# codebydant/sfM_danPipeline

Measured on AMD Instinct MI355X. Metric: image-pairs matched/sec + BA iterations/sec (200 cams, 100k pts, 1M obs), higher is better.
Workload: dtype i8

## Files before the change

### sfm_danpipeline_amd/csrc/match.hip

```cpp
#include "common.h"
#include <type_traits>
#include <vector>
#include <algorithm>
#include <string.h>
#include <stdlib.h>

namespace {

typedef int v4i __attribute__((ext_vector_type(4)));
typedef int v16i __attribute__((ext_vector_type(16)));

enum { KIND_F32_L2 = 0, KIND_U8_L2 = 1, KIND_U8_HAMMING = 2 };

constexpr int TILE_ROWS = 32;
constexpr int HPAD = -(1 << 23);
constexpr int TAG_BITS = 8;
constexpr int EPOCH_TILES = 1 << TAG_BITS;
constexpr int TAG_MASK = EPOCH_TILES - 1;
constexpr int FIX_FLAG = 1 << 30;
constexpr int FIX_GRID = 1024;
constexpr int FIX_CAP = 1 << 20;
constexpr int DIST_EMPTY = 0x7FFFFFFF;
constexpr int KNN_WAVES = 4;
constexpr int HCHUNK = 1024;
// ... 192 lines not shown
      }
    }
#pragma unroll
    for (int e = 0; e < 16; ++e) {
      const int k = c * 16 + e;
      int x = 128;
      if (valid && k < dim) {
        if (KIND == KIND_F32_L2) {
          const float f = fv[e];
          ok = ok && (f == rintf(f)) && (f >= 0.f) && (f <= 255.f);
          x = (int)f;
          x = x < 0 ? 0 : (x > 255 ? 255 : x);
        } else {
          x = bv[e];
        }
      }
      const int cv = x - 128;
      v[e] = (signed char)cv;
      n2 += cv * cv;
    }
  }
#pragma unroll
  for (int o = 1; o < NC; o <<= 1) n2 += __shfl_xor(n2, o);
  int4 out;
  memcpy(&out, v, 16);
  int4* dst = (int4*)(I.tiles + (size_t)tile * (TILE_ROWS * RB)) + chunk_pos<NC>(r, c);
  *dst = out;
  if (c == 0) {
    int ci;
    if (KIND == KIND_U8_HAMMING)
      ci = ((valid ? dim * 8 * (HCHUNK / 2) : (dim * 8 + 1) * HCHUNK)) | (pos & (HCHUNK - 1));
    else ci = valid ? -((n2 + 1) >> 1) : HPAD;
    I.cin[pos] = ci;
    I.nq[pos] = valid ? n2 : 0;
  }
  if (KIND == KIND_F32_L2 && !ok) nonintegral[img] = gen;
}

template <int NC>
__device__ __forceinline__ int group_sum(int x) {
  if (NC >= 2) x += __builtin_amdgcn_update_dpp(0, x, 0xB1, 0xF, 0xF, true);
  if (NC >= 4) x += __builtin_amdgcn_update_dpp(0, x, 0x4E, 0xF, 0xF, true);
  if (NC >= 8) x += __builtin_amdgcn_update_dpp(0, x, 0x141, 0xF, 0xF, true);
  if (NC >= 16) x += __builtin_amdgcn_update_dpp(0, x, 0x140, 0xF, 0xF, true);
  return x;
}

struct Best2 {
  int d0, i0, x0, d1, i1, x1;
};
__device__ __forceinline__ bool lex_less(int da, int ia, int db, int ib) { return da < db || (da == db && ia < ib); }
__device__ __forceinline__ void best2_insert(Best2& b, int d, int i, int x) {
  if (lex_less(d, i, b.d0, b.i0)) {
    b.d1 = b.d0;
    b.i1 = b.i0;
    b.x1 = b.x0;
    b.d0 = d;
    b.i0 = i;
    b.x0 = x;
  } else if (lex_less(d, i, b.d1, b.i1)) {
    b.d1 = d;
    b.i1 = i;
    b.x1 = x;
  }
}

template <int I>
__device__ __forceinline__ void epi_op(const v16i& D0, const v16i& D1, int (&sl)[16], int& k0, int& k1, int (&T)[16],
                                       int tag0, int tag1) {
  if constexpr (I < 16) {
    sl[I] = imax3(sl[I], D0[I], D1[I]);
  } else {
    constexpr int J = (I - 16) % 11;
    constexpr int B = (I - 16) < 11 ? 0 : 8;
    const v16i& D = (I - 16) < 11 ? D0 : D1;
    const int tag = (I - 16) < 11 ? tag0 : tag1;
    if constexpr (J == 0) T[B + 0] = imax3(D[0], D[1], D[2]);
    if constexpr (J == 1) T[B + 1] = imax3(D[3], D[4], D[5]);
    if constexpr (J == 2) T[B + 2] = imax3(D[6], D[7], D[8]);
    if constexpr (J == 3) T[B + 3] = imax3(D[9], D[10], D[11]);
    if constexpr (J == 4) T[B + 4] = imax3(D[12], D[13], D[14]);
    if constexpr (J == 5) T[B + 5] = imax3(T[B + 0], T[B + 1], T[B + 2]);
    if constexpr (J == 6) T[B + 6] = imax3(T[B + 3], T[B + 4], D[15]);
    if constexpr (J == 7) T[B + 7] = max(T[B + 5], T[B + 6]);
    if constexpr (J == 8) T[B + 7] = (T[B + 7] << TAG_BITS) | tag;
    if constexpr (J == 9) k1 = imed3(k0, k1, T[B + 7]);
    if constexpr (J == 10) k0 = max(k0, T[B + 7]);
  }
}
constexpr int EPI_ORDER[38] = {16, 17, 18, 19, 20, 21, 22, 23, 24, 25, 26, 27, 28, 29, 30, 31, 0, 1,  2,
                                          32, 33, 3,  4,  5,  34, 6,  7,  8,  9,  35, 10, 11, 12, 13, 36, 37, 14, 15};
template <int LO, int HI>
__device__ __forceinline__ void epi_range(const v16i& D0, const v16i& D1, int (&sl)[16], int& k0, int& k1, int (&T)[16],
                                          int tag0, int tag1) {
  if constexpr (LO < HI && LO < 38) {
    epi_op<EPI_ORDER[LO]>(D0, D1, sl, k0, k1, T, tag0, tag1);
    epi_range<LO + 1, HI>(D0, D1, sl, k0, k1, T, tag0, tag1);
  }
}

template <int KS, int MODE, int NU, int SR>
__global__ __launch_bounds__(KNN_WAVES * 64, 2) void knn_kernel(const ImgDev* __restrict__ imgs,
                                                         const WorkItem* __restrict__ items,
                                                         const int* __restrict__ nonintegral, int gen, int dim,
                                                         int4* __restrict__ knn, int maxq,
                                                         int* __restrict__ fix_count, int2* __restrict__ fix_items) {
  constexpr int NC = 2 * KS;
  constexpr int RB = 32 * KS;
  constexpr int TILE_BYTES = TILE_ROWS * RB;
  constexpr int STAGE_ROW_BYTES = SR * RB;
  constexpr int NW = KNN_WAVES;
  constexpr int NT = NW * 64;
  constexpr int CIN_COPIES = (SR + NT - 1) / NT;
  constexpr int STAGE_BYTES = STAGE_ROW_BYTES + CIN_COPIES * NT * 4;
  constexpr int TILES = SR / TILE_ROWS;
  constexpr int TP = TILES / 2;
  constexpr int PIECES = STAGE_ROW_BYTES / (NT * 16);
  constexpr int BATCH = KS <= 4 ? 4 : 2;
  constexpr int NG = 2 * KS;
  constexpr int STAGES_PER_EPOCH = EPOCH_TILES / TILES;
  static_assert(PIECES >= 1 && TP >= 2 && TP % 2 == 0 && STAGES_PER_EPOCH % 2 == 0, "stage shape");
  constexpr int SCRATCH_W = 2048 + (TILE_ROWS * RB > 4096 ? TILE_ROWS * RB : 4096);
  constexpr int BUFA_BYTES = STAGE_BYTES > NW * SCRATCH_W ? STAGE_BYTES : NW * SCRATCH_W;
  constexpr int BUFB_BYTES = (NU < 2 || STAGE_BYTES > NW * SCRATCH_W) ? STAGE_BYTES : NW * SCRATCH_W;
  __shared__ __attribute__((aligned(16))) unsigned char ldsA[BUFA_BYTES];
  __shared__ __attribute__((aligned(16))) unsigned char ldsB[BUFB_BYTES];

  const WorkItem it = items[blockIdx.x];
  if ((nonintegral[it.qimg] == gen) | (nonintegral[it.timg] == gen)) return;
  const ImgDev Q = imgs[it.qimg];
  const ImgDev T = imgs[it.timg];
  const int lane = threadIdx.x & 63;
  const int wave = __builtin_amdgcn_readfirstlane(threadIdx.x >> 6);
  const int r = lane & 31, h = lane >> 5;
  const int nqt = Q.n_pad / TILE_ROWS;
  int qt[NU], qtc[NU];
#pragma unroll
  for (int u = 0; u < NU; ++u) {
    qt[u] = it.qtile0 + NU * wave + u;
    qtc[u] = qt[u] < Q.n_pad / TILE_ROWS ? qt[u] : (Q.n_pad >= TILE_ROWS ? Q.n_pad / TILE_ROWS - 1 : 0);
  }
  SFM_STAMP(0);
  int dbg_trips = 0;

  v4i bq[NU][KS];
#pragma unroll
  for (int u = 0; u < NU; ++u) {
    g_v4i_p src = (g_v4i_p)(Q.tiles + (size_t)qtc[u] * TILE_BYTES);
#pragma unroll
    for (int ks = 0; ks < KS; ++ks) bq[u][ks] = src[chunk_pos<NC>(r, 2 * ks + h)];
  }

  int aoff[KS];
#pragma unroll
  for (int ks = 0; ks < KS; ++ks) aoff[ks] = chunk_pos<NC>(r, 2 * ks + h) * 16;
  const int coff = STAGE_ROW_BYTES + h * 16;

  const int nstages = T.n_pad / SR;
  const int tid = threadIdx.x;

  const __amdgpu_buffer_rsrc_t rs_tiles = __builtin_amdgcn_make_buffer_rsrc((void*)T.tiles, 0, 0x7FFFFFFF, 0x00020000);
  const __amdgpu_buffer_rsrc_t rs_cin = __builtin_amdgcn_make_buffer_rsrc((void*)T.cin, 0, 0x7FFFFFFF, 0x00020000);
  auto stage_copy = [&](int stage, unsigned char* dstb) {
    const int off = stage * STAGE_ROW_BYTES;
#if SFM_DBG == 6
    const unsigned char* src = (const unsigned char*)T.tiles + (size_t)stage * STAGE_ROW_BYTES;
#pragma unroll
    for (int i = 0; i < PIECES; ++i)
      __builtin_amdgcn_global_load_lds((const SFM_GLOBAL void*)(src + (size_t)(i * NT + tid) * 16),
                                       (__attribute__((address_space(3))) void*)(dstb + i * (NT * 16) + wave * 1024), 16, 0, 0);
#pragma unroll
    for (int i = 0; i < CIN_COPIES; ++i)
      __builtin_amdgcn_global_load_lds((const SFM_GLOBAL void*)(T.cin + (size_t)stage * SR + i * NT + tid),
                                       (__attribute__((address_space(3))) void*)(dstb + STAGE_ROW_BYTES + i * (NT * 4) + wave * 256), 4, 0, 0);
    (void)off;
#else
#pragma unroll
    for (int i = 0; i < PIECES; ++i)
      __builtin_amdgcn_raw_ptr_buffer_load_lds(rs_tiles, (__attribute__((address_space(3))) void*)(dstb + i * (NT * 16) + wave * 1024),
                                               16, (i * NT + tid) * 16, off, 0, 0);
#pragma unroll
    for (int i = 0; i < CIN_COPIES; ++i)
      __builtin_amdgcn_raw_ptr_buffer_load_lds(rs_cin, (__attribute__((address_space(3))) void*)(dstb + STAGE_ROW_BYTES + i * (NT * 4) + wave * 256),
                                               4, (i * NT + tid) * 4, stage * SR * 4, 0, 0);
#endif
  };
  auto ld_afrag = [&](const unsigned char* tb, int ks) -> v4i {
    const int4 x = *(const int4*)(tb + aoff[ks]);
    return v4i{x.x, x.y, x.z, x.w};
  };
  auto ld_cin = [&](const unsigned char* sb, int tl, v16i& C) {
#pragma unroll
    for (int g = 0; g < 4; ++g) {
      const int4 x = *(const int4*)(sb + coff + (tl * TILE_ROWS + 8 * g) * 4);
      C[4 * g] = x.x;
      C[4 * g + 1] = x.y;
      C[4 * g + 2] = x.z;
      C[4 * g + 3] = x.w;
    }
  };

  const int nodd_t = MODE == 0 ? *(g_i32_p)T.nodd : 0;
  const int nbits = dim * 8;

  for (int ep0 = 0; ep0 < nstages; ep0 += STAGES_PER_EPOCH) {
    const int ep1 = (ep0 + STAGES_PER_EPOCH < nstages) ? ep0 + STAGES_PER_EPOCH : nstages;
    const int ep_tile0 = ep0 * TILES;
    int sl[NU][16], k0[NU], k1[NU];
#pragma unroll
    for (int u = 0; u < NU; ++u) {
      k0[u] = k1[u] = (int)0x80000000;
#pragma unroll
      for (int e = 0; e < 16; ++e) sl[u][e] = HPAD;
    }
    if (ep0 > 0) __syncthreads();
    stage_copy(ep0, ldsA);
    asm volatile("s_waitcnt vmcnt(0)" ::: "memory");
    __syncthreads();

    v4i F0[KS], F1[KS];
    v16i C0, C1, X0, X1, Y0, Y1;
    int TT[16];
    {
      const unsigned char* sb = ldsA;
#pragma unroll
      for (int ks = 0; ks < KS; ++ks) F0[ks] = ld_afrag(sb, ks);
      ld_cin(sb, 0, C0);
#pragma unroll
      for (int e = 0; e < 16; ++e) X0[e] = X1[e] = Y0[e] = Y1[e] = HPAD;
    }
    int tag = EPOCH_TILES - 1 + 2;
    SFM_STAMP(1);

#define SFM_CHAIN(FA, FB, UF, DA, DB, UD, LD1, SB1, T1, LD0, SB0, T0)                                       \
  do {                                                                                                      \
    _Pragma("unroll") for (int g_ = 0; g_ < NG; ++g_) {                                                     \
      const int ks_ = g_ % KS;                                                                              \
      if (SFM_DBG == 3) {                                                                                   \
        if (g_ < KS) FA[ks_] += F0[ks_][0] + C0[ks_];                                                       \
        else FB[ks_] += F1[ks_][0] + C1[ks_];                                                               \
      } else if (g_ < KS) FA = __builtin_amdgcn_mfma_i32_32x32x32_i8(F0[ks_], bq[UF][ks_], ks_ == 0 ? C0 : FA, 0, 0, 0); \
      else FB = __builtin_amdgcn_mfma_i32_32x32x32_i8(F1[ks_], bq[UF][ks_], ks_ == 0 ? C1 : FB, 0, 0, 0);  \
      if ((LD1) && g_ == 0) {                                                                               \
        _Pragma("unroll") for (int k2_ = 0; k2_ < KS; ++k2_) F1[k2_] = ld_afrag((SB1) + (T1) * TILE_BYTES, k2_); \
        ld_cin(SB1, T1, C1);                                                                                \
      }                                                                                                     \
      if ((LD0) && g_ < KS) {                                                                               \
        F0[ks_] = ld_afrag((SB0) + (T0) * TILE_BYTES, ks_);                                                 \
        if (g_ == 0) ld_cin(SB0, T0, C0);                                                                   \
      }                                                                                                     \
      if (SFM_DBG != 2) switch (g_) {                                                                       \
        SFM_EPI_CASES(DA, DB, UD)                                                                           \
      }                                                                                                     \
      __builtin_amdgcn_sched_barrier(0);                                                                    \
    }                                                                                                       \
  } while (0)
#define SFM_EPI_CASE(G, DA, DB, UD) \
  case G: epi_range<(G) * 38 / NG, ((G) + 1) * 38 / NG>(DA, DB, sl[UD], k0[UD], k1[UD], TT, tag & TAG_MASK, (tag - 1) & TAG_MASK); break;
#define SFM_EPI_CASES(DA, DB, UD)                                                                          \
  SFM_EPI_CASE(0, DA, DB, UD) SFM_EPI_CASE(1, DA, DB, UD) SFM_EPI_CASE(2, DA, DB, UD) SFM_EPI_CASE(3, DA, DB, UD)     \
  SFM_EPI_CASE(4, DA, DB, UD) SFM_EPI_CASE(5, DA, DB, UD) SFM_EPI_CASE(6, DA, DB, UD) SFM_EPI_CASE(7, DA, DB, UD)     \
  SFM_EPI_CASE(8, DA, DB, UD) SFM_EPI_CASE(9, DA, DB, UD) SFM_EPI_CASE(10, DA, DB, UD) SFM_EPI_CASE(11, DA, DB, UD)   \
  SFM_EPI_CASE(12, DA, DB, UD) SFM_EPI_CASE(13, DA, DB, UD) SFM_EPI_CASE(14, DA, DB, UD) SFM_EPI_CASE(15, DA, DB, UD)

    auto stage = [&](int s, const unsigned char* sb, unsigned char* nb) __attribute__((always_inline)) {
      const bool more = s + 1 < ep1;
      if (more) stage_copy(s + 1, nb);
#pragma unroll
      for (int tp = 0; tp < TP; ++tp) {
        const bool last = tp == TP - 1;
        if (NU == 2) {
          SFM_CHAIN(X0, X1, 0, Y0, Y1, 1, true, sb, 2 * tp + 1, false, sb, 0);
          tag -= 2;
          if (last) {
            asm volatile("s_waitcnt vmcnt(0)" ::: "memory");
            __syncthreads();
          }
          SFM_CHAIN(Y0, Y1, NU - 1, X0, X1, 0, false, sb, 0, true, last ? nb : sb, last ? 0 : 2 * tp + 2);
        } else {
          if (last) {
#pragma unroll
            for (int k2 = 0; k2 < KS; ++k2) F1[k2] = ld_afrag(sb + (2 * tp + 1) * TILE_BYTES, k2);
            ld_cin(sb, 2 * tp + 1, C1);
            asm volatile("s_waitcnt vmcnt(0)" ::: "memory");
            __syncthreads();
          }
          if ((tp & 1) == 0) SFM_CHAIN(X0, X1, 0, Y0, Y1, 0, !last, sb, 2 * tp + 1, true, last ? nb : sb, last ? 0 : 2 * tp + 2);
          else SFM_CHAIN(Y0, Y1, 0, X0, X1, 0, !last, sb, 2 * tp + 1, true, last ? nb : sb, last ? 0 : 2 * tp + 2);
          tag -= 2;
        }
      }
    
    };
    for (int s = ep0; s < ep1; s += 2) {
      stage(s, ldsA, ldsB);
      if (s + 1 < ep1) stage(s + 1, ldsB, ldsA);
    }
    SFM_STAMP(2);
    epi_range<0, 38>(Y0, Y1, sl[NU - 1], k0[NU - 1], k1[NU - 1], TT, tag & TAG_MASK, (tag - 1) & TAG_MASK);
#undef SFM_CHAIN
#undef SFM_EPI_CASES
#undef SFM_EPI_CASE

    int lane_p = lane;
    asm volatile("" : "+v"(lane_p));
    const int r_p = lane_p & 31, h_p = lane_p >> 5;
    typedef __attribute__((address_space(3))) int* lds_vi_p;
#define SFM_WAVE_LDS_FENCE() do { __builtin_amdgcn_fence(__ATOMIC_RELEASE, "wavefront"); __builtin_amdgcn_wave_barrier(); __builtin_amdgcn_fence(__ATOMIC_ACQUIRE, "wavefront"); } while (0)
    __attribute__((address_space(3))) unsigned char* wq[NU];
#pragma unroll
    for (int u = 0; u < NU; ++u)
      wq[u] = (__attribute__((address_space(3))) unsigned char*)(u == 0 ? ldsA : ldsB) + wave * SCRATCH_W + 2048;
    const lds_vi_p wl = (lds_vi_p)(wq[0] - 2048);
    const lds_vi_p wr = NU == 1 ? wl + 256 : (lds_vi_p)(wq[NU - 1] - 2048);
#pragma unroll
    for (int u = 0; u < NU; ++u)
#pragma unroll
      for (int ks = 0; ks < KS; ++ks)
        *(__attribute__((address_space(3))) v4i*)(wq[u] + chunk_pos<NC>(r_p, 2 * ks + h_p) * 16) = bq[u][ks];
    constexpr int SH = (NC == 16) ? 0 : (NC == 8) ? 1 : (NC == 4) ? 2 : 3;
    int cpos[NU][4], chv[NU][4], slot_[NU][4], count[NU];
    bool cval[NU][4], cload[NU][4];
    int qrow[NU], nqq[NU];
    int ovf[NU];
#pragma unroll
    for (int u = 0; u < NU; ++u) {
      const int q = qtc[u] * TILE_ROWS + r_p;
      qrow[u] = ((g_i32_p)Q.perm)[q];
      nqq[u] = ((g_i32_p)Q.nq)[q];
      if (qt[u] >= nqt) qrow[u] = -1;
    }
#pragma unroll
    for (int u = 0; u < NU; ++u) {
      const int bv0 = k0[u] >> TAG_BITS, bv1 = k1[u] >> TAG_BITS;
      const int tl0 = ep_tile0 + (EPOCH_TILES - 1) - (k0[u] & TAG_MASK);
      const int tl1 = ep_tile0 + (EPOCH_TILES - 1) - (k1[u] & TAG_MASK);
      const int pb0 = __shfl_xor(bv0, 32), pb1 = __shfl_xor(bv1, 32);
      int a0 = (HPAD - 1) * 16, a1 = a0, a2 = a0;
#pragma unroll
      for (int e = 0; e < 16; ++e) {
        const int key = (int)((unsigned)sl[u][e] << 4) | e;
        a2 = imed3(a1, a2, key);
        a1 = imed3(a0, a1, key);
        a0 = max(a0, key);
      }
      const int S0 = a0 >> 4, S1 = a1 >> 4, S2 = a2 >> 4;
      const int e0 = a0 & 15, e1 = a1 & 15;
      const int thr = max(max(min(bv0, pb0), max(bv1, pb1)), S1);
      const int ns = (S0 >= thr ? 1 : 0) + (S1 >= thr ? 1 : 0) + (S2 >= thr ? 1 : 0);
      const bool t0in = bv0 >= thr && bv0 > HPAD, t1in = bv1 >= thr && bv1 > HPAD;
      const int rho0 = 8 * (e0 >> 2) + 4 * h_p + (e0 & 3), rho1 = ns >= 2 ? 8 * (e1 >> 2) + 4 * h_p + (e1 & 3) : rho0;
      int over = (ns > 2 && (t0in || t1in)) ? 1 : 0;
      over |= __shfl_xor(over, 32);
      ovf[u] = over;
      const bool known = ns == 1;
      cpos[u][0] = tl0 * TILE_ROWS + rho0;
      cpos[u][1] = tl0 * TILE_ROWS + rho1;
      cpos[u][2] = tl1 * TILE_ROWS + rho0;
      cpos[u][3] = tl1 * TILE_ROWS + rho1;
      cval[u][0] = t0in && ns >= 1;
      cval[u][1] = t0in && ns >= 2;
      cval[u][2] = t1in && ns >= 1;
      cval[u][3] = t1in && ns >= 2;
      chv[u][0] = known ? bv0 : HPAD - 1;
      chv[u][1] = HPAD - 1;
      chv[u][2] = known ? bv1 : HPAD - 1;
      chv[u][3] = HPAD - 1;
      bool need[4] = {!known, !known, !known, !known};
#if SFM_RESOLVE_V2
      if (ns == 2 && S0 != S1 && t0in) {
        const bool gt = S1 > bv1, eq = S1 == bv1, lt = S1 < bv1;
        const bool e1_in = gt || (eq && tl0 < tl1);
        const bool first0 = rho0 < rho1;
        cval[u][0] = true, chv[u][0] = bv0, need[0] = false;
        cval[u][1] = e1_in, chv[u][1] = S1, need[1] = e1_in && !gt;
        cval[u][2] = eq || lt, chv[u][2] = bv1, need[2] = eq && first0;
        cval[u][3] = eq, chv[u][3] = bv1, need[3] = eq && !first0;
      }
#endif
#pragma unroll
      for (int k = 0; k < 4; ++k) {
        cval[u][k] = cval[u][k] && cpos[u][k] < T.n_pad;
        cload[u][k] = cval[u][k] && need[k] && SFM_DBG != 1;
      }
    }
    SFM_STAMP(8);
    int total = 0;
#pragma unroll
    for (int u = 0; u < NU; ++u) {
#pragma unroll
      for (int k = 0; k < 4; ++k) {
        const unsigned long long bm = __ballot(cload[u][k]);
        slot_[u][k] = total + __popcll(bm & ((1ull << lane_p) - 1ull));
        if (cload[u][k]) wl[slot_[u][k]] = cpos[u][k] | (r_p << 26) | (u << 31);
        total += __popcll(bm);
      }
      count[u] = total;
    }
    SFM_WAVE_LDS_FENCE();
    SFM_STAMP(9);
#if SFM_DBG == 4
    if (blockIdx.x < 4096 && lane == 0) {
      g_stamps[(blockIdx.x * 8 + wave) * 16 + 13] = count[0];
      g_stamps[(blockIdx.x * 8 + wave) * 16 + 7] = total - count[0];
    }
#endif
    {
      constexpr int LPR = NC >= 2 ? NC / 2 : 1;
      constexpr int CPL = NC / LPR;
      constexpr int RPS = 64 / LPR;
      constexpr int STEPS = 64 / RPS;
      const int grp = lane_p / LPR, c = lane_p % LPR;
      auto trip = [&](int j0, auto ns_) __attribute__((always_inline)) {
        constexpr int NS = decltype(ns_)::value;
        v4i xt[NS][CPL], xq[NS][CPL];
        int ci[NS];
#pragma unroll
        for (int st = 0; st < NS; ++st) {
          const int j = j0 + st * RPS + grp;
          unsigned ent = (unsigned)wl[j & (NU * 256 - 1)];
          if (j >= total) ent = 0u;
          const unsigned ps = ent & ((1u << 26) - 1u), qr = (ent >> 26) & 31u;
          const unsigned x = ((ps >> SH) ^ (qr >> SH)) & (unsigned)(NC - 1);
          const unsigned char* trow = (const unsigned char*)T.tiles + ps * (unsigned)RB;
          const __attribute__((address_space(3))) unsigned char* qrw = ((NU > 1 && (ent >> 31)) ? wq[NU - 1] : wq[0]) + qr * (unsigned)RB;
#pragma unroll
          for (int i = 0; i < CPL; ++i) {
            const unsigned p_ = (unsigned)(c + i * LPR);
            xt[st][i] = *(g_v4i_p)(trow + p_ * 16);
            xq[st][i] = *(const __attribute__((address_space(3))) v4i*)(qrw + ((p_ ^ x) << 4));
          }
          ci[st] = ((g_i32_p)T.cin)[ps];
        }
        SFM_STAMP(11);
#if SFM_DBG == 4
        asm volatile("s_waitcnt vmcnt(0)" ::: "memory");
        SFM_STAMP(12);
#endif
#pragma unroll
        for (int st = 0; st < NS; ++st) {
          int dot = 0;
#pragma unroll
          for (int i = 0; i < CPL; ++i)
#pragma unroll
            for (int w = 0; w < 4; ++w) dot = __builtin_amdgcn_sdot4(xt[st][i][w], xq[st][i][w], dot, false);
          dot = group_sum<LPR>(dot) + ci[st];
          wr[(j0 + st * RPS + grp) & (NU * 256 - 1)] = dot;
        }
      };
      for (int j0 = 0; j0 < total; j0 += RPS * STEPS) {
        ++dbg_trips;
        const int left = total - j0;
        if (STEPS >= 4 && left <= RPS * (STEPS / 4)) trip(j0, std::integral_constant<int, (STEPS >= 4 ? STEPS / 4 : 1)>{});
        else if (STEPS >= 2 && left <= RPS * (STEPS / 2)) trip(j0, std::integral_constant<int, (STEPS >= 2 ? STEPS / 2 : 1)>{});
        else if (STEPS >= 4 && left <= RPS * (3 * STEPS / 4)) trip(j0, std::integral_constant<int, (STEPS >= 4 ? 3 * STEPS / 4 : 1)>{});
        else trip(j0, std::integral_constant<int, STEPS>{});
      }
    }
    SFM_WAVE_LDS_FENCE();
    SFM_STAMP(10);
    long long lane_dk[NU][2];
#pragma unroll
    for (int u = 0; u < NU; ++u) {
      long long key[4];
#pragma unroll
      for (int k = 0; k < 4; ++k) {
        if (cload[u][k]) chv[u][k] = wr[slot_[u][k]];
        const int hv = cval[u][k] ? chv[u][k] : HPAD - 1;
        key[k] = ((long long)hv << 32) | (unsigned)(0x7FFFFFFF - cpos[u][k]);
      }
      const long long a = max(key[0], key[1]), b = min(key[0], key[1]);
      const long long c = max(key[2], key[3]), dd = min(key[2], key[3]);
      const long long lk[2] = {max(a, c), max(min(a, c), max(b, dd))};
#pragma unroll
      for (int k = 0; k < 2; ++k) {
        const int hv = (int)(lk[k] >> 32), ps = 0x7FFFFFFF - (int)(unsigned)lk[k];
        const int d = MODE == 0 ? nqq[u] - 2 * hv - (ps < nodd_t ? 1 : 0) : (nbits - hv) >> 1;
        lane_dk[u][k] = hv > HPAD ? (((long long)d << 32) | (unsigned)ps) : 0x7FFFFFFFFFFFFFFFll;
      }
    }
    constexpr bool SPLIT = NU == 2;
    const bool um = SPLIT && h_p != 0;
    long long mine[2], give[2];
#pragma unroll
    for (int k = 0; k < 2; ++k) {
      mine[k] = um ? lane_dk[NU - 1][k] : lane_dk[0][k];
      give[k] = SPLIT ? (um ? lane_dk[0][k] : lane_dk[NU - 1][k]) : lane_dk[0][k];
    }
    const long long o0 = __shfl_xor(give[0], 32), o1 = __shfl_xor(give[1], 32);
    const long long best0 = min(mine[0], o0), best1 = min(max(mine[0], o0), min(mine[1], o1));
    const int my_qrow = um ? qrow[NU - 1] : qrow[0];
    int my_ovf = um ? ovf[NU - 1] : ovf[0];
    const unsigned p0 = (unsigned)best0, p1 = (unsigned)best1;
    const int px0 = ((g_i32_p)T.perm)[p0 < (unsigned)T.n_pad ? p0 : 0u];
    const int px1 = ((g_i32_p)T.perm)[p1 < (unsigned)T.n_pad ? p1 : 0u];
    {
      Best2 m;
      m.d0 = (int)(best0 >> 32), m.i0 = (int)(unsigned)best0, m.x0 = px0;
      m.d1 = (int)(best1 >> 32), m.i1 = (int)(unsigned)best1, m.x1 = px1;
      if (best0 == 0x7FFFFFFFFFFFFFFFll || m.x0 < 0) m.d0 = DIST_EMPTY, m.i0 = 0x7FFFFFFF, m.x0 = -1;
      if (best1 == 0x7FFFFFFFFFFFFFFFll || m.x1 < 0) m.d1 = DIST_EMPTY, m.i1 = 0x7FFFFFFF, m.x1 = -1;
      if ((SPLIT || h_p == 0) && my_qrow >= 0) {
        int4* dst = &knn[(size_t)it.pair * maxq + my_qrow];
        if (ep0 > 0) {
          const int4 pv = *dst;
          Best2 a;
          a.d0 = pv.z, a.x0 = pv.x, a.i0 = -2, a.d1 = pv.w, a.x1 = pv.y, a.i1 = -1;
          if (pv.y == FIX_FLAG) my_ovf = 1;
          if (m.d0 != DIST_EMPTY) best2_insert(a, m.d0, m.i0, m.x0);
          if (m.d1 != DIST_EMPTY) best2_insert(a, m.d1, m.i1, m.x1);
          m = a;
        }
        int4 o;
        if (ep1 < nstages) {
          o.x = m.x0;
          o.y = my_ovf ? FIX_FLAG : m.x1;
          o.z = m.d0;
          o.w = m.d1;
        } else {
          const bool v0 = m.d0 != DIST_EMPTY, v1 = m.d1 != DIST_EMPTY;
          float d0, d1;
          int fix = 0;
          if (MODE == 0) {
            d0 = sqrtf((float)m.d0);
            d1 = sqrtf((float)m.d1);
            if (v1 && m.d1 >= (1 << 22)) fix = FIX_FLAG;
          } else {
            d0 = (float)m.d0;
            d1 = (float)m.d1;
          }
          o.x = v0 ? m.x0 : -1;
          o.y = v1 ? (m.x1 | fix) : -1;
          if (my_ovf) o.y = FIX_FLAG;
          o.z = __float_as_int(v0 ? d0 : 3.402823466e+38f);
          o.w = __float_as_int(v1 ? d1 : 3.402823466e+38f);
          if (o.y >= 0 && (o.y & FIX_FLAG)) {
            const int k = atomicAdd(fix_count, 1);
            if (k < FIX_CAP) fix_items[k] = make_int2(it.pair, my_qrow);
          }
        }
        *dst = o;
      }
    }
    SFM_STAMP(3);
    SFM_STAMP(4);
  }

  SFM_STAMP(5);
#if SFM_DBG == 4
  if (blockIdx.x < 4096 && lane == 0) {
    g_stamps[(blockIdx.x * 8 + wave) * 16 + 14] = __builtin_amdgcn_s_getreg((4 << 0) | (0 << 6) | (31 << 11));
    g_stamps[(blockIdx.x * 8 + wave) * 16 + 15] = __builtin_amdgcn_s_getreg((20 << 0) | (0 << 6) | (31 << 11));
  }
  if (blockIdx.x < 4096 && lane == 0) g_stamps[(blockIdx.x * 8 + wave) * 16 + 6] = dbg_trips;
#endif
}

constexpr int HIB = 10;
static_assert((1 << HIB) == HCHUNK, "the key's index bits");
constexpr unsigned KEY_EMPTY = 0xFFFFFFFFu;
__device__ __forceinline__ unsigned umin_(unsigned a, unsigned b) { return a < b ? a : b; }
__device__ __forceinline__ unsigned umax_(unsigned a, unsigned b) { return a > b ? a : b; }
struct Top2 {
  unsigned s0, s1;
  int j0, j1;
};

__device__ __forceinline__ void chunk_merge(Top2& g, unsigned k0, unsigned k1, int cb) {
  const unsigned ns0 = k0 >> HIB, ns1 = k1 >> HIB;
  const int nj0 = cb + (int)(k0 & (HCHUNK - 1)), nj1 = cb + (int)(k1 & (HCHUNK - 1));
  const bool e0 = (k0 == KEY_EMPTY), e1 = (k1 == KEY_EMPTY);
  const unsigned a0 = e0 ? KEY_EMPTY : ns0, a1 = e1 ? KEY_EMPTY : ns1;
  if (a0 < g.s0) {
    if (a1 < g.s0) {
      g.s1 = a1;
      g.j1 = nj1;
    } else {
      g.s1 = g.s0;
      g.j1 = g.j0;
    }
    g.s0 = a0;
    g.j0 = nj0;
  } else if (a0 < g.s1) {
    g.s1 = a0;
    g.j1 = nj0;
  }
}

__device__ __forceinline__ bool lex_less_u(unsigned sa, int ja, unsigned sb, int jb) {
  return sa < sb || (sa == sb && ja < jb);
}

template <int KS, int SR>
__global__ __launch_bounds__(256, 2) void knn_keyed_kernel(const ImgDev* __restrict__ imgs,
                                                           const WorkItem* __restrict__ items, int dim,
                                                           int4* __restrict__ knn, int maxq) {
  constexpr int MODE = 1;
  constexpr int NC = 2 * KS;
  constexpr int RB = 32 * KS;
  constexpr int STAGE_ROW_BYTES = SR * RB;
  constexpr int STAGE_BYTES = STAGE_ROW_BYTES + SR * 4;
  constexpr int TILES = SR / TILE_ROWS;
  constexpr int PIECES = STAGE_ROW_BYTES / 4096;
  constexpr int HALF = PIECES > 1 ? PIECES / 2 : 1;
  __shared__ __attribute__((aligned(16))) unsigned char ldsA[STAGE_BYTES];
  __shared__ __attribute__((aligned(16))) unsigned char ldsB[STAGE_BYTES];

  const WorkItem it = items[blockIdx.x];
  const ImgDev Q = imgs[it.qimg];
  const ImgDev T = imgs[it.timg];
  const int lane = threadIdx.x & 63;
  const int wave = __builtin_amdgcn_readfirstlane(threadIdx.x >> 6);
  const int r = lane & 31, h = lane >> 5;
  const int nqt = (Q.n_rows + TILE_ROWS - 1) / TILE_ROWS;
  const int qt[2] = {it.qtile0 + 2 * wave, it.qtile0 + 2 * wave + 1};

  v4i bq[2][KS];
#pragma unroll
  for (int u = 0; u < 2; ++u) {
    const int t = qt[u] < nqt ? qt[u] : (nqt > 0 ? nqt - 1 : 0);
    g_v4i_p src = (g_v4i_p)(Q.tiles + (size_t)t * (TILE_ROWS * RB));
#pragma unroll
    for (int ks = 0; ks < KS; ++ks) {
      v4i x = src[chunk_pos<NC>(r, 2 * ks + h)];
#pragma unroll
      for (int w = 0; w < 4; ++w) {
        const unsigned neg = (unsigned)x[w] ^ (((unsigned)x[w] & 0x08080808u) * 30u);
        x[w] = (int)((neg << 3) & 0xC0C0C0C0u);
      }
      bq[u][ks] = x;
    }
  }

  int aoff[KS];
#pragma unroll
  for (int ks = 0; ks < KS; ++ks) aoff[ks] = chunk_pos<NC>(r, 2 * ks + h) * 16;
  const int boff = STAGE_ROW_BYTES + h * 16;

  Top2 g[2];
  unsigned k0[2], k1[2];
#pragma unroll
  for (int u = 0; u < 2; ++u) {
    g[u].s0 = g[u].s1 = KEY_EMPTY;
    g[u].j0 = g[u].j1 = -1;
    k0[u] = k1[u] = KEY_EMPTY;
  }

  const int nstages = T.n_pad / SR;
  const int tid = threadIdx.x;

  const __amdgpu_buffer_rsrc_t rs_tiles = __builtin_amdgcn_make_buffer_rsrc((void*)T.tiles, 0, 0x7FFFFFFF, 0x00020000);
  const __amdgpu_buffer_rsrc_t rs_cin = __builtin_amdgcn_make_buffer_rsrc((void*)T.cin, 0, 0x7FFFFFFF, 0x00020000);
  auto stage_copy = [&](int stage, unsigned char* dstb) {
    const int off = stage * STAGE_ROW_BYTES;
#pragma unroll
    for (int i = 0; i < PIECES; ++i)
      __builtin_amdgcn_raw_ptr_buffer_load_lds(rs_tiles, (__attribute__((address_space(3))) void*)(dstb + i * 4096 + wave * 1024), 16,
                                               (i * 256 + tid) * 16, off, 0, 0);
    if (wave < SR / 64)
      __builtin_amdgcn_raw_ptr_buffer_load_lds(rs_cin, (__attribute__((address_space(3))) void*)(dstb + STAGE_ROW_BYTES + wave * 256), 4,
                                               tid * 4, stage * SR * 4, 0, 0);
  };

  stage_copy(0, ldsA);
  asm volatile("s_waitcnt vmcnt(0)" ::: "memory");
  __syncthreads();

#define SFM_MFMA(ACC, FR, u, ks, BS) \
  ACC = __builtin_amdgcn_mfma_i32_32x32x32_i8(FR[ks], bq[u][ks], (ks) == 0 ? BS : ACC, 0, 0, 0)
#define SFM_INS(ACC, u, e)                                                             \
  do {                                                                                     \
    const unsigned key_ = (unsigned)ACC[e];                  \
    const unsigned n1_ = umax_(umin_(k0[u], k1[u]), umin_(umax_(k0[u], k1[u]), key_));  \
    k0[u] = umin_(k0[u], key_);                                                            \
    k1[u] = n1_;                                                                           \
    asm volatile("" : "+v"(k0[u]), "+v"(k1[u]));  \
  } while (0)
  auto ld_afrag = [&](const unsigned char* sb, int tl, int ks) -> v4i {
    const int4 x = *(const int4*)(sb + tl * (TILE_ROWS * RB) + aoff[ks]);
    return v4i{x.x, x.y, x.z, x.w};
  };
  auto ld_bases = [&](const unsigned char* sb, int tl, int gq, v16i& bs) {
    const int4 x = *(const int4*)(sb + boff + (tl * TILE_ROWS + 8 * gq) * 4);
    bs[4 * gq] = x.x;
    bs[4 * gq + 1] = x.y;
    bs[4 * gq + 2] = x.z;
    bs[4 * gq + 3] = x.w;
  };

  constexpr int MPG = (KS + 3) / 4;
#define SFM_GROUP(g_, SB, tl, CA0, CA1, NA0, NA1, FN, FNN, BC, BN, do_mfma, do_frag)              \
  do {                                                                                         \
    if (do_mfma) {                                                                             \
      _Pragma("unroll") for (int j_ = 0; j_ < MPG; ++j_) {                                     \
        const int ks_ = ((g_) & 3) * MPG + j_;                                                 \
        if (ks_ < KS) {                                                                        \
          if ((g_) < 4) SFM_MFMA(NA0, FN, 0, ks_, BN);                                         \
          else SFM_MFMA(NA1, FN, 1, ks_, BN);                                                  \
        }                                                                                      \
      }                                                                                        \
      if ((g_) >= 4) {                                                                         \
        if (do_frag) ld_bases(SB, (tl) + 2, (g_) - 4, BC);  \
      }                                                                                        \
      else if (do_frag) {                                                                      \
        _Pragma("unroll") for (int j_ = 0; j_ < MPG; ++j_)                                     \
          if ((g_) * MPG + j_ < KS) FNN[(g_) * MPG + j_] = ld_afrag(SB, (tl) + 2, (g_) * MPG + j_); \
      }                                                                                        \
    }                                                                                          \
    SFM_INS(CA0, 0, 2 * (g_));                                                                 \
    SFM_INS(CA1, 1, 2 * (g_));                                                                 \
    SFM_INS(CA0, 0, 2 * (g_) + 1);                                                             \
    SFM_INS(CA1, 1, 2 * (g_) + 1);                                                             \
    __builtin_amdgcn_sched_barrier(0);                                                         \
  } while (0)
#define SFM_BODY(SB, tl, CA0, CA1, NA0, NA1, FN, FNN, BC, BN, mf_, fr_)                        \
  do {                                                                                         \
    SFM_GROUP(0, SB, tl, CA0, CA1, NA0, NA1, FN, FNN, BC, BN, mf_, fr_);                       \
    SFM_GROUP(1, SB, tl, CA0, CA1, NA0, NA1, FN, FNN, BC, BN, mf_, fr_);                       \
    SFM_GROUP(2, SB, tl, CA0, CA1, NA0, NA1, FN, FNN, BC, BN, mf_, fr_);                       \
    SFM_GROUP(3, SB, tl, CA0, CA1, NA0, NA1, FN, FNN, BC, BN, mf_, fr_);                       \
    SFM_GROUP(4, SB, tl, CA0, CA1, NA0, NA1, FN, FNN, BC, BN, mf_, fr_);                       \
    SFM_GROUP(5, SB, tl, CA0, CA1, NA0, NA1, FN, FNN, BC, BN, mf_, fr_);                       \
    SFM_GROUP(6, SB, tl, CA0, CA1, NA0, NA1, FN, FNN, BC, BN, mf_, fr_);                       \
    SFM_GROUP(7, SB, tl, CA0, CA1, NA0, NA1, FN, FNN, BC, BN, mf_, fr_);                       \
  } while (0)

  static_assert(TILES == 4 || TILES == 8, "stage = 4 or 8 train tiles");
  v4i fa[KS], fb[KS];
  v16i ba, bb;
  v16i A0, A1, B0, B1;
#pragma unroll
  for (int ks = 0; ks < KS; ++ks) fa[ks] = ld_afrag(ldsA, 0, ks);
#pragma unroll
  for (int gq = 0; gq < 4; ++gq) ld_bases(ldsA, 0, gq, ba);
#pragma unroll
  for (int gq = 0; gq < 4; ++gq) ld_bases(ldsA, 1, gq, bb);
#pragma unroll
  for (int ks = 0; ks < KS; ++ks) SFM_MFMA(A0, fa, 0, ks, ba);
#pragma unroll
  for (int ks = 0; ks < KS; ++ks) SFM_MFMA(A1, fa, 1, ks, ba);
#pragma unroll
  for (int ks = 0; ks < KS; ++ks) fb[ks] = ld_afrag(ldsA, 1, ks);
  __builtin_amdgcn_sched_barrier(0);

  auto stage = [&](int s, const unsigned char* sb, unsigned char* nb) __attribute__((always_inline)) {
    const bool more = s + 1 < nstages;
    if (more) stage_copy(s + 1, nb);

    SFM_BODY(sb, 0, A0, A1, B0, B1, fb, fa, ba, bb, true, true);
    SFM_BODY(sb, 1, B0, B1, A0, A1, fa, fb, bb, ba, true, true);
    if (TILES == 8) {
      SFM_BODY(sb, 2, A0, A1, B0, B1, fb, fa, ba, bb, true, true);
      SFM_BODY(sb, 3, B0, B1, A0, A1, fa, fb, bb, ba, true, true);
      SFM_BODY(sb, 4, A0, A1, B0, B1, fb, fa, ba, bb, true, true);
      SFM_BODY(sb, 5, B0, B1, A0, A1, fa, fb, bb, ba, true, true);
    }
    SFM_BODY(sb, TILES - 2, A0, A1, B0, B1, fb, fa, ba, bb, true, false);
    asm volatile("s_waitcnt vmcnt(0)" ::: "memory");
    __syncthreads();
    if (more) {
#pragma unroll
      for (int ks = 0; ks < KS; ++ks) fa[ks] = ld_afrag(nb, 0, ks);
#pragma unroll
      for (int gq = 0; gq < 4; ++gq) ld_bases(nb, 0, gq, ba);
    }
    SFM_BODY(nb, -1, B0, B1, A0, A1, fa, fb, bb, ba, more, more);
    if (((s + 1) * SR) % HCHUNK == 0) {
      const int cb = ((s * SR) / HCHUNK) * HCHUNK;
#pragma unroll
      for (int u = 0; u < 2; ++u) {
        chunk_merge(g[u], k0[u], k1[u], cb);
        k0[u] = k1[u] = KEY_EMPTY;
      }
    }
  };
  for (int s = 0; s < nstages; s += 2) {
    stage(s, ldsA, ldsB);
    if (s + 1 < nstages) stage(s + 1, ldsB, ldsA);
  }
  if ((nstages * SR) % HCHUNK != 0) {
    const int cb = ((nstages * SR) / HCHUNK) * HCHUNK;
#pragma unroll
    for (int u = 0; u < 2; ++u) chunk_merge(g[u], k0[u], k1[u], cb);
  }
#undef SFM_BODY
#undef SFM_GROUP
#undef SFM_INS
#undef SFM_MFMA

#pragma unroll
  for (int u = 0; u < 2; ++u) {
    Top2 p;
    p.s0 = __shfl_xor(g[u].s0, 32);
    p.s1 = __shfl_xor(g[u].s1, 32);
    p.j0 = __shfl_xor(g[u].j0, 32);
    p.j1 = __shfl_xor(g[u].j1, 32);
    Top2 m;
    if (lex_less_u(p.s0, p.j0, g[u].s0, g[u].j0)) {
      m.s0 = p.s0;
      m.j0 = p.j0;
      if (lex_less_u(g[u].s0, g[u].j0, p.s1, p.j1)) {
        m.s1 = g[u].s0;
        m.j1 = g[u].j0;
      } else {
        m.s1 = p.s1;
// ... 1136 lines not shown
```

Measured before the change: 2.080 million.

## Merge dual-query-tile epilogue into one lane set via permlane32 swap

When two query tiles are processed per wave, the epilogue now swaps per-lane score and key registers across wave halves with permlane32_swap, so each lane holds both halves of a single query row. The top-2 selection, candidate resolution and rescoring then run once per lane instead of once per tile followed by cross-half shuffles. This removes duplicated top-3 scans, the per-tile ballot/compaction loops and several shfl_xor exchanges. The price is a more intricate merge of the key pairs, where tag and tie handling must stay exactly equivalent to the old path.

Result: slower. 1.990 million (-4.4%).

```diff
diff --git a/sfm_danpipeline_amd/csrc/match.hip b/sfm_danpipeline_amd/csrc/match.hip
--- a/sfm_danpipeline_amd/csrc/match.hip
+++ b/sfm_danpipeline_amd/csrc/match.hip
@@ -518,9 +518,22 @@
 #undef SFM_EPI_CASES
 #undef SFM_EPI_CASE
 
+    constexpr bool MERGED = NU == 2;
+    if constexpr (MERGED) {
+      auto swap32 = [](int& a, int& b) __attribute__((always_inline)) {
+        const auto x = __builtin_amdgcn_permlane32_swap((unsigned)a, (unsigned)b, false, false);
+        a = (int)x[0];
+        b = (int)x[1];
+      };
+#pragma unroll
+      for (int e = 0; e < 16; ++e) swap32(sl[0][e], sl[NU - 1][e]);
+      swap32(k0[0], k0[NU - 1]);
+      swap32(k1[0], k1[NU - 1]);
+    }
     int lane_p = lane;
     asm volatile("" : "+v"(lane_p));
     const int r_p = lane_p & 31, h_p = lane_p >> 5;
+    const bool um = MERGED && h_p != 0;
     typedef __attribute__((address_space(3))) int* lds_vi_p;
 #define SFM_WAVE_LDS_FENCE() do { __builtin_amdgcn_fence(__ATOMIC_RELEASE, "wavefront"); __builtin_amdgcn_wave_barrier(); __builtin_amdgcn_fence(__ATOMIC_ACQUIRE, "wavefront"); } while (0)
     __attribute__((address_space(3))) unsigned char* wq[NU];
@@ -535,90 +548,122 @@
       for (int ks = 0; ks < KS; ++ks)
         *(__attribute__((address_space(3))) v4i*)(wq[u] + chunk_pos<NC>(r_p, 2 * ks + h_p) * 16) = bq[u][ks];
     constexpr int SH = (NC == 16) ? 0 : (NC == 8) ? 1 : (NC == 4) ? 2 : 3;
-    int cpos[NU][4], chv[NU][4], slot_[NU][4], count[NU];
-    bool cval[NU][4], cload[NU][4];
-    int qrow[NU], nqq[NU];
-    int ovf[NU];
-#pragma unroll
-    for (int u = 0; u < NU; ++u) {
-      const int q = qtc[u] * TILE_ROWS + r_p;
-      qrow[u] = ((g_i32_p)Q.perm)[q];
-      nqq[u] = ((g_i32_p)Q.nq)[q];
-      if (qt[u] >= nqt) qrow[u] = -1;
-    }
-#pragma unroll
-    for (int u = 0; u < NU; ++u) {
-      const int bv0 = k0[u] >> TAG_BITS, bv1 = k1[u] >> TAG_BITS;
-      const int tl0 = ep_tile0 + (EPOCH_TILES - 1) - (k0[u] & TAG_MASK);
-      const int tl1 = ep_tile0 + (EPOCH_TILES - 1) - (k1[u] & TAG_MASK);
-      const int pb0 = __shfl_xor(bv0, 32), pb1 = __shfl_xor(bv1, 32);
-      int a0 = (HPAD - 1) * 16, a1 = a0, a2 = a0;
-#pragma unroll
-      for (int e = 0; e < 16; ++e) {
-        const int key = (int)((unsigned)sl[u][e] << 4) | e;
+    constexpr int UH = MERGED ? 2 : 1;
+    constexpr int SLOT_BITS = MERGED ? 5 : 4;
+    int cpos[4], chv[4], slot_[4];
+    bool cval[4], cload[4];
+    const int my_qt = um ? qt[NU - 1] : qt[0], my_qtc = um ? qtc[NU - 1] : qtc[0];
+    int my_qrow = ((g_i32_p)Q.perm)[my_qtc * TILE_ROWS + r_p];
+    const int nqq = ((g_i32_p)Q.nq)[my_qtc * TILE_ROWS + r_p];
+    if (my_qt >= nqt) my_qrow = -1;
+    int my_ovf;
+    {
+      int K0, K1, hi2;
+      if constexpr (MERGED) {
+        const int ka0 = k0[0], ka1 = k1[0], kb0 = k0[1], kb1 = k1[1];
+        const bool atop = ka0 >= kb0, same = ((ka0 ^ kb0) & TAG_MASK) == 0;
+        const int lo0 = min(ka0, kb0);
+        K0 = max(ka0, kb0);
+        K1 = max(atop ? ka1 : kb1, same ? (atop ? kb1 : ka1) : lo0);
+        hi2 = max(lo0, max(ka1, kb1)) >> TAG_BITS;
+      } else {
+        K0 = k0[0], K1 = k1[0];
+        const int pb0 = __shfl_xor(K0 >> TAG_BITS, 32), pb1 = __shfl_xor(K1 >> TAG_BITS, 32);
+        hi2 = max(min(K0 >> TAG_BITS, pb0), max(K1 >> TAG_BITS, pb1));
+      }
+      const int bv0 = K0 >> TAG_BITS, bv1 = K1 >> TAG_BITS;
+      const int tl0 = ep_tile0 + (EPOCH_TILES - 1) - (K0 & TAG_MASK);
+      const int tl1 = ep_tile0 + (EPOCH_TILES - 1) - (K1 & TAG_MASK);
+      int t3[UH][3];
+#pragma unroll
+      for (int hh = 0; hh < UH; ++hh) t3[hh][0] = t3[hh][1] = t3[hh][2] = (HPAD - 1) * (1 << SLOT_BITS);
+#pragma unroll
+      for (int e = 0; e < 16; ++e)
+#pragma unroll
+        for (int hh = 0; hh < UH; ++hh) {
+          const int key = (int)((unsigned)sl[hh][e] << SLOT_BITS) | (hh * 16 + e);
+          t3[hh][2] = imed3(t3[hh][1], t3[hh][2], key);
+          t3[hh][1] = imed3(t3[hh][0], t3[hh][1], key);
+          t3[hh][0] = max(t3[hh][0], key);
+        }
+      int a0 = t3[0][0], a1 = t3[0][1], a2 = t3[0][2];
+#pragma unroll
+      for (int j = 0; j < (MERGED ? 3 : 0); ++j) {
+        const int key = t3[UH - 1][j];
         a2 = imed3(a1, a2, key);
         a1 = imed3(a0, a1, key);
         a0 = max(a0, key);
       }
-      const int S0 = a0 >> 4, S1 = a1 >> 4, S2 = a2 >> 4;
-      const int e0 = a0 & 15, e1 = a1 & 15;
-      const int thr = max(max(min(bv0, pb0), max(bv1, pb1)), S1);
+      const int S0 = a0 >> SLOT_BITS, S1 = a1 >> SLOT_BITS, S2 = a2 >> SLOT_BITS;
+      const int e0 = a0 & ((1 << SLOT_BITS) - 1), e1 = a1 & ((1 << SLOT_BITS) - 1);
+      const int thr = max(hi2, S1);
       const int ns = (S0 >= thr ? 1 : 0) + (S1 >= thr ? 1 : 0) + (S2 >= thr ? 1 : 0);
       const bool t0in = bv0 >= thr && bv0 > HPAD, t1in = bv1 >= thr && bv1 > HPAD;
-      const int rho0 = 8 * (e0 >> 2) + 4 * h_p + (e0 & 3), rho1 = ns >= 2 ? 8 * (e1 >> 2) + 4 * h_p + (e1 & 3) : rho0;
+      auto slot_row = [&](int s) { return 8 * ((s & 15) >> 2) + 4 * (MERGED ? s >> 4 : h_p) + (s & 3); };
+      const int rho0 = slot_row(e0), rho1 = ns >= 2 ? slot_row(e1) : rho0;
       int over = (ns > 2 && (t0in || t1in)) ? 1 : 0;
-      over |= __shfl_xor(over, 32);
-      ovf[u] = over;
+      if constexpr (!MERGED) over |= __shfl_xor(over, 32);
+      my_ovf = over;
       const bool known = ns == 1;
-      cpos[u][0] = tl0 * TILE_ROWS + rho0;
-      cpos[u][1] = tl0 * TILE_ROWS + rho1;
-      cpos[u][2] = tl1 * TILE_ROWS + rho0;
-      cpos[u][3] = tl1 * TILE_ROWS + rho1;
-      cval[u][0] = t0in && ns >= 1;
-      cval[u][1] = t0in && ns >= 2;
-      cval[u][2] = t1in && ns >= 1;
-      cval[u][3] = t1in && ns >= 2;
-      chv[u][0] = known ? bv0 : HPAD - 1;
-      chv[u][1] = HPAD - 1;
-      chv[u][2] = known ? bv1 : HPAD - 1;
-      chv[u][3] = HPAD - 1;
+      cpos[0] = tl0 * TILE_ROWS + rho0;
+      cpos[1] = tl0 * TILE_ROWS + rho1;
+      cpos[2] = tl1 * TILE_ROWS + rho0;
+      cpos[3] = tl1 * TILE_ROWS + rho1;
+      cval[0] = t0in && ns >= 1;
+      cval[1] = t0in && ns >= 2;
+      cval[2] = t1in && ns >= 1;
+      cval[3] = t1in && ns >= 2;
+      chv[0] = known ? bv0 : HPAD - 1;
+      chv[1] = HPAD - 1;
+      chv[2] = known ? bv1 : HPAD - 1;
+      chv[3] = HPAD - 1;
       bool need[4] = {!known, !known, !known, !known};
 #if SFM_RESOLVE_V2
       if (ns == 2 && S0 != S1 && t0in) {
         const bool gt = S1 > bv1, eq = S1 == bv1, lt = S1 < bv1;
         const bool e1_in = gt || (eq && tl0 < tl1);
         const bool first0 = rho0 < rho1;
-        cval[u][0] = true, chv[u][0] = bv0, need[0] = false;
-        cval[u][1] = e1_in, chv[u][1] = S1, need[1] = e1_in && !gt;
-        cval[u][2] = eq || lt, chv[u][2] = bv1, need[2] = eq && first0;
-        cval[u][3] = eq, chv[u][3] = bv1, need[3] = eq && !first0;
+        cval[0] = true, chv[0] = bv0, need[0] = false;
+        cval[1] = e1_in, chv[1] = S1, need[1] = e1_in && !gt;
+        cval[2] = eq || lt, chv[2] = bv1, need[2] = eq && first0;
+        cval[3] = eq, chv[3] = bv1, need[3] = eq && !first0;
       }
 #endif
+      if constexpr (MERGED) {
+        if (ns == 2 && ((e0 ^ e1) & 16)) {
+          const bool x1 = (e0 & 16) != 0;
+          const int kc[4] = {x1 ? k0[NU - 1] : k0[0], x1 ? k1[NU - 1] : k1[0], x1 ? k0[0] : k0[NU - 1], x1 ? k1[0] : k1[NU - 1]};
+#pragma unroll
+          for (int k = 0; k < 4; ++k) {
+            const int v = kc[k] >> TAG_BITS;
+            cpos[k] = (ep_tile0 + (EPOCH_TILES - 1) - (kc[k] & TAG_MASK)) * TILE_ROWS + (k < 2 ? rho0 : rho1);
+            cval[k] = v >= thr && v > HPAD;
+            chv[k] = v;
+            need[k] = false;
+          }
+        }
+      }
 #pragma unroll
       for (int k = 0; k < 4; ++k) {
-        cval[u][k] = cval[u][k] && cpos[u][k] < T.n_pad;
-        cload[u][k] = cval[u][k] && need[k] && SFM_DBG != 1;
+        cval[k] = cval[k] && cpos[k] < T.n_pad;
+        cload[k] = cval[k] && need[k] && SFM_DBG != 1;
       }
     }
     SFM_STAMP(8);
     int total = 0;
 #pragma unroll
-    for (int u = 0; u < NU; ++u) {
-#pragma unroll
-      for (int k = 0; k < 4; ++k) {
-        const unsigned long long bm = __ballot(cload[u][k]);
-        slot_[u][k] = total + __popcll(bm & ((1ull << lane_p) - 1ull));
-        if (cload[u][k]) wl[slot_[u][k]] = cpos[u][k] | (r_p << 26) | (u << 31);
-        total += __popcll(bm);
-      }
-      count[u] = total;
+    for (int k = 0; k < 4; ++k) {
+      const unsigned long long bm = __ballot(cload[k]);
+      slot_[k] = total + __popcll(bm & ((1ull << lane_p) - 1ull));
+      if (cload[k]) wl[slot_[k]] = cpos[k] | (r_p << 26) | ((um ? 1 : 0) << 31);
+      total += __popcll(bm);
     }
     SFM_WAVE_LDS_FENCE();
     SFM_STAMP(9);
 #if SFM_DBG == 4
     if (blockIdx.x < 4096 && lane == 0) {
-      g_stamps[(blockIdx.x * 8 + wave) * 16 + 13] = count[0];
-      g_stamps[(blockIdx.x * 8 + wave) * 16 + 7] = total - count[0];
+      g_stamps[(blockIdx.x * 8 + wave) * 16 + 13] = total;
+      g_stamps[(blockIdx.x * 8 + wave) * 16 + 7] = 0;
     }
 #endif
     {
@@ -675,15 +720,14 @@
     }
     SFM_WAVE_LDS_FENCE();
     SFM_STAMP(10);
-    long long lane_dk[NU][2];
-#pragma unroll
-    for (int u = 0; u < NU; ++u) {
+    long long dk[2];
+    {
       long long key[4];
 #pragma unroll
       for (int k = 0; k < 4; ++k) {
-        if (cload[u][k]) chv[u][k] = wr[slot_[u][k]];
-        const int hv = cval[u][k] ? chv[u][k] : HPAD - 1;
-        key[k] = ((long long)hv << 32) | (unsigned)(0x7FFFFFFF - cpos[u][k]);
+        if (cload[k]) chv[k] = wr[slot_[k]];
+        const int hv = cval[k] ? chv[k] : HPAD - 1;
+        key[k] = ((long long)hv << 32) | (unsigned)(0x7FFFFFFF - cpos[k]);
       }
       const long long a = max(key[0], key[1]), b = min(key[0], key[1]);
       const long long c = max(key[2], key[3]), dd = min(key[2], key[3]);
@@ -691,22 +735,17 @@
 #pragma unroll
       for (int k = 0; k < 2; ++k) {
         const int hv = (int)(lk[k] >> 32), ps = 0x7FFFFFFF - (int)(unsigned)lk[k];
-        const int d = MODE == 0 ? nqq[u] - 2 * hv - (ps < nodd_t ? 1 : 0) : (nbits - hv) >> 1;
-        lane_dk[u][k] = hv > HPAD ? (((long long)d << 32) | (unsigned)ps) : 0x7FFFFFFFFFFFFFFFll;
-      }
-    }
-    constexpr bool SPLIT = NU == 2;
-    const bool um = SPLIT && h_p != 0;
-    long long mine[2], give[2];
-#pragma unroll
-    for (int k = 0; k < 2; ++k) {
-      mine[k] = um ? lane_dk[NU - 1][k] : lane_dk[0][k];
-      give[k] = SPLIT ? (um ? lane_dk[0][k] : lane_dk[NU - 1][k]) : lane_dk[0][k];
-    }
-    const long long o0 = __shfl_xor(give[0], 32), o1 = __shfl_xor(give[1], 32);
-    const long long best0 = min(mine[0], o0), best1 = min(max(mine[0], o0), min(mine[1], o1));
-    const int my_qrow = um ? qrow[NU - 1] : qrow[0];
-    int my_ovf = um ? ovf[NU - 1] : ovf[0];
+        const int d = MODE == 0 ? nqq - 2 * hv - (ps < nodd_t ? 1 : 0) : (nbits - hv) >> 1;
+        dk[k] = hv > HPAD ? (((long long)d << 32) | (unsigned)ps) : 0x7FFFFFFFFFFFFFFFll;
+      }
+    }
+    long long best0, best1;
+    if constexpr (MERGED) {
+      best0 = min(dk[0], dk[1]), best1 = max(dk[0], dk[1]);
+    } else {
+      const long long o0 = __shfl_xor(dk[0], 32), o1 = __shfl_xor(dk[1], 32);
+      best0 = min(dk[0], o0), best1 = min(max(dk[0], o0), min(dk[1], o1));
+    }
     const unsigned p0 = (unsigned)best0, p1 = (unsigned)best1;
     const int px0 = ((g_i32_p)T.perm)[p0 < (unsigned)T.n_pad ? p0 : 0u];
     const int px1 = ((g_i32_p)T.perm)[p1 < (unsigned)T.n_pad ? p1 : 0u];
@@ -716,7 +755,7 @@
       m.d1 = (int)(best1 >> 32), m.i1 = (int)(unsigned)best1, m.x1 = px1;
       if (best0 == 0x7FFFFFFFFFFFFFFFll || m.x0 < 0) m.d0 = DIST_EMPTY, m.i0 = 0x7FFFFFFF, m.x0 = -1;
       if (best1 == 0x7FFFFFFFFFFFFFFFll || m.x1 < 0) m.d1 = DIST_EMPTY, m.i1 = 0x7FFFFFFF, m.x1 = -1;
-      if ((SPLIT || h_p == 0) && my_qrow >= 0) {
+      if ((MERGED || h_p == 0) && my_qrow >= 0) {
         int4* dst = &knn[(size_t)it.pair * maxq + my_qrow];
         if (ep0 > 0) {
           const int4 pv = *dst;
```
